# mlcolab/Pathfinder.jl

Hardware: AMD Instinct MI355X
Metric: ELBO draws/sec (multipathfinder hot path: fit + ELBO + pool + PSIS + resample) (higher is better)
Workload: dtype f64

## Files before the change

pathfinder.jl_amd/csrc/elbo_qf_kernel.hip:

```cpp
#include <type_traits>
#include <stdio.h>
#include <stdlib.h>
#include "pfmi_common.h"
#include "elbo_args.h"
#ifndef QF_PROF
#define QF_PROF 0
#endif

#ifndef QF_WAVES
#define QF_WAVES 8
#endif
#define QF_THREADS (QF_WAVES * 64)
#ifndef QF_NG
#define QF_NG 2
#endif
#ifndef QF_ABLATE
#define QF_ABLATE 0
#endif
#ifndef QF_NG2_MAXKC
#define QF_NG2_MAXKC 20
#endif
#ifndef QF_PRIO_FAIR
#define QF_PRIO_FAIR 8
#endif
#ifndef QF_PRIO_YOUNG
#define QF_PRIO_YOUNG 0
#endif
#ifndef QF_SETPRIO
#define QF_SETPRIO 0
#endif
#define QF_MIN_FRONT 1024
static_assert(QF_MIN_FRONT >= 2 * PF_ICDF_BFE_FRONT, "the look-up's front guard");
template <int KC> struct qf_chb { static constexpr int v = (KC > 20) ? 8 : 16; };

#pragma clang fp contract(off)

typedef double qf_d4 __attribute__((ext_vector_type(4)));
__device__ __forceinline__ qf_d4 qf_mfma16(double a, double b, qf_d4 c) { return __builtin_amdgcn_mfma_f64_16x16x4f64(a, b, c, 0, 0, 0); }
__device__ __forceinline__ double qf_mfma4(double a, double b, double c) { return __builtin_amdgcn_mfma_f64_4x4x4f64(a, b, c, 0, 0, 0); }

__host__ __device__ constexpr int qf_nconst(int KC, int RPAD) { return 4 + KC + KC * KC + RPAD + RPAD * KC + KC; }

template <int TGT>
__device__ __forceinline__ void qf_row_ac(const ElboArgs &A, const double *mu, int i, double &a, double &c) {
    if (TGT == 1) { a = A.t_a[i]; c = mu[i] - A.t_mean[i]; }
    else if (TGT == 2) { a = (i >= 1) ? 1.0 : 0.0; c = mu[i]; }
    else { a = 0.0; c = 0.0; }
}

template <int KC>
__device__ __forceinline__ int qf_vh_pos(int lrow, int col) {
    const int bl = lrow >> 4, rr = lrow & 15, q = rr >> 2, r = rr & 3, T = col >> 2, i = col & 3;
    return (((bl * 4 + r) * (KC / 4) + T) << 4) + q * 4 + i;
}

struct QfKernArgs { ElboArgs A; int ch_blocks, nchunks, groups_per_wg, ngroups, n_whole, n_tail, ndep; double *cshare; unsigned *cflag; unsigned epoch; };
#ifndef QF_SHARE_SPINS
#define QF_SHARE_SPINS 2000000
#endif
template <int KC, int TGT, int RPAD, int NG>
__global__ __launch_bounds__(QF_THREADS) void pf_elbo_qf_kernel(ElboArgs A, int ch_blocks, int nchunks, int groups_per_wg, int ngroups, int n_whole,
                                                                  int n_tail, int ndep, double *, unsigned *, unsigned) {
    extern __shared__ __attribute__((aligned(16))) double lds[];
#if QF_PROF
    const long long qf_t0 = wall_clock64();
    long long qf_tb = 0, qf_te = 0, qf_tp = 0, qf_last = 0;
#endif
    constexpr int NT = KC / 4, TR = RPAD / 4, NC = qf_nconst(KC, RPAD);
    constexpr int QF_CHB = qf_chb<KC>::v;
    constexpr bool FOLD = !(NG == 2 && KC >= 16);
    constexpr int PRE = (QF_CHB * 16 * KC + QF_THREADS - 1) / QF_THREADS;
    const int tid = threadIdx.x, wv = tid >> 6, lane = tid & 63, q = lane >> 4, c = lane & 15, l3 = lane & 3;
    const int d = A.d, nblk = (d + 15) >> 4;
    int slot = blockIdx.y, role = 0;
    int g_begin = blockIdx.x * groups_per_wg, g_cap = groups_per_wg;
    if (n_tail > 0 && slot >= n_whole) {
        constexpr int SL = QF_WAVES * NG, NPG_ = (TGT != 0) ? (KC + 1 + 15) / 16 : 0;
        int tail_f;
        if (slot < n_whole + n_tail) { role = 1; tail_f = slot - n_whole; g_begin = 0; g_cap = SL - NPG_; }
        else {
            const int t = slot - n_whole - n_tail;
            role = 2; tail_f = t / ndep;
            g_begin = (SL - NPG_) + (t - tail_f * ndep) * SL; g_cap = SL;
        }
        slot = n_whole + tail_f;
    }
    const int p = A.points[slot];
    const size_t blkidx = A.by_point ? (size_t)p : (size_t)slot;
    double *out_lp = A.logp + blkidx * A.log_stride, *out_lq = A.logq + blkidx * A.log_stride;
    constexpr int NPG = (TGT != 0) ? (KC + 1 + 15) / 16 : 0;
    const int npg = (role == 2) ? 0 : NPG;
    const int g_end = (g_begin + g_cap < ngroups) ? g_begin + g_cap : ngroups;
    const int nlb = (npg + (g_end - g_begin) + QF_WAVES * NG - 1) / (QF_WAVES * NG);
    if (A.status[p] != PFMI_FIT_OK) {
        for (int64_t n = (int64_t)g_begin * 16 + tid; n < (int64_t)g_end * 16 && n < A.N; n += QF_THREADS) {
            out_lp[n] = NAN; out_lq[n] = NAN;
        }
        return;
    }
    const int vh_sz = ch_blocks * 16 * KC, rs_sz = ch_blocks * 48;
    const int buf_stride = (nchunks > 1) ? vh_sz + rs_sz : 0;
    const int stage_sz = (nchunks > 1 ? 2 : 1) * (vh_sz + rs_sz);
    const int fix_off = stage_sz > QF_MIN_FRONT ? stage_sz : QF_MIN_FRONT;
    double *t_s = lds + fix_off;
    double *cn_s = t_s + KC * KC;
    double *g_s = cn_s + NC;
    double2 *icdf = reinterpret_cast<double2 *>(g_s + RPAD * RPAD + ((KC * KC + NC + RPAD * RPAD) & 1));

    const double *Vh = A.vh + (size_t)p * d * KC, *mu = A.mu + (size_t)p * d, *sqa = A.sqrt_alpha + (size_t)p * d;
    auto stage_direct = [&](int ck, int buf) {
        const int row0 = ck * ch_blocks * 16;
        double *vs = lds + buf * buf_stride, *rs = vs + vh_sz;
        const int npair = ch_blocks * 8 * KC;
        const int lim = (d - row0) * KC;
        const double2 *src = reinterpret_cast<const double2 *>(Vh + (size_t)row0 * KC);
        constexpr int U = 6;
        for (int j0 = tid; j0 < npair; j0 += QF_THREADS * U) {
            double2 v[U];
#pragma unroll
            for (int u = 0; u < U; ++u) {
                const int j = j0 + u * QF_THREADS, jc = (2 * j + 1 < lim) ? j : (lim >> 1) - 1;
                v[u] = src[jc];
            }
#pragma unroll
            for (int u = 0; u < U; ++u) {
                const int j = j0 + u * QF_THREADS, idx = 2 * j;
                if (j < npair) {
                    const int lrow = idx / KC, col = idx - lrow * KC;
                    const double2 val = (idx < lim) ? v[u] : make_double2(0.0, 0.0);
                    *reinterpret_cast<double2 *>(vs + qf_vh_pos<KC>(lrow, col)) = val;
                }
            }
        }
        for (int l0 = tid; l0 < ch_blocks * 16; l0 += QF_THREADS * 2) {
            double a[2], cc[2], s[2];
#pragma unroll
            for (int u = 0; u < 2; ++u) {
                const int lrow = l0 + u * QF_THREADS, row = row0 + lrow, rc = row < d ? row : d - 1;
                qf_row_ac<TGT>(A, mu, rc, a[u], cc[u]);
                s[u] = sqa[rc];
            }
#pragma unroll
            for (int u = 0; u < 2; ++u) {
                const int lrow = l0 + u * QF_THREADS, row = row0 + lrow;
                if (lrow < ch_blocks * 16) {
                    const bool in = row < d;
                    double *o = rs + (lrow >> 4) * 48 + (lrow & 15);
                    o[0] = in ? a[u] * s[u] * s[u] : 0.0; o[16] = in ? 2.0 * a[u] * cc[u] * s[u] : 0.0; o[32] = in ? s[u] : 0.0;
                }
            }
        }
    };
    {
        const double *T = A.tmat + (size_t)p * KC * KC;
        for (int i = tid; i < KC * KC; i += QF_THREADS) t_s[i] = T[i];
        for (int i = tid; i < NC; i += QF_THREADS) cn_s[i] = 0.0;
        if (RPAD > 0) for (int i = tid; i < RPAD * RPAD; i += QF_THREADS) g_s[i] = A.t_g[i];
        pf_icdf_load(icdf);
        stage_direct(0, 0);
    }
    const int rho = 4 * (c & 3) + (c >> 2);
    constexpr bool HREG = !(NG == 2 && KC >= 16);
    const double *Vc = A.vchol + (size_t)p * KC * KC;
    auto head_op = [&](const int which, const int r) -> double {
        const int b = 4 * q + r;
        if (which == 0) { double v = (rho == b) ? 1.0 : 0.0; if (rho < KC && b < KC) v = Vc[b * KC + rho]; return v; }
        const int i1 = 16 + rho, b1 = 16 + b;
        if (which == 1) return (i1 < KC) ? Vc[b * KC + i1] : 0.0;
        double v1 = (i1 == b1) ? 1.0 : 0.0;
        if (i1 < KC && b1 < KC) v1 = Vc[b1 * KC + i1];
        return v1;
    };
    double a_h00[HREG ? 4 : 1], a_h10[HREG ? 4 : 1], a_h11[HREG ? 4 : 1];
    if (HREG) {
#pragma unroll
        for (int r = 0; r < 4; ++r) {
            a_h00[HREG ? r : 0] = head_op(0, r);
            a_h10[HREG ? r : 0] = (KC > 16) ? head_op(1, r) : 0.0;
            a_h11[HREG ? r : 0] = (KC > 16) ? head_op(2, r) : 0.0;
        }
    }
    auto hop = [&](const int which, const int r) -> double {
        if (HREG) return which == 0 ? a_h00[HREG ? r : 0] : (which == 1 ? a_h10[HREG ? r : 0] : a_h11[HREG ? r : 0]);
        return head_op(which, r);
    };
    const uint64_t seed = A.seeds[slot];
    const uint32_t k0 = (uint32_t)seed, k1 = (uint32_t)(seed >> 32);
    const double logdet = A.logdet[p];
    __syncthreads();
#if QF_PROF
    qf_tp = wall_clock64() - qf_t0; qf_last = wall_clock64();
#endif
#if QF_PRIO_YOUNG
    if (wv >= 4) __builtin_amdgcn_s_setprio(1);
#endif
    if (TGT == 2) {
        if (tid == 0) { cn_s[1] = mu[0]; cn_s[2] = sqa[0]; }
        if (tid < KC) cn_s[4 + KC + KC * KC + RPAD + RPAD * KC + tid] = Vh[tid];
    }

    int cur = 0;
    for (int lb = 0; lb < nlb; ++lb) {
        bool pseudo[NG], active[NG];
        int sl[NG];
        int64_t nl[NG];
        uint32_t n[NG];
        double accw[NG][NT], acc3[NG][NT], acc4[NG][TR > 0 ? TR : 1];
        double usq[NG], q12[NG], z00[NG], u0[NG][4];
        bool any_active = false, any_pseudo = false, any_real = false;
#pragma unroll
        for (int g = 0; g < NG; ++g) {
            sl[g] = (lb * QF_WAVES + wv) * NG + g;
            pseudo[g] = sl[g] < npg;
            const int grp = g_begin + sl[g] - npg;
            active[g] = pseudo[g] || grp < g_end;
            nl[g] = (int64_t)grp * 16 + c;
            n[g] = (uint32_t)(A.n0 + nl[g]);
            any_active |= active[g]; any_pseudo |= pseudo[g]; any_real |= active[g] && !pseudo[g];
#pragma unroll
            for (int T = 0; T < NT; ++T) { accw[g][T] = 0.0; acc3[g][T] = 0.0; }
#pragma unroll
            for (int T = 0; T < (TR > 0 ? TR : 1); ++T) acc4[g][T] = 0.0;
            usq[g] = 0.0; q12[g] = 0.0; z00[g] = 0.0;
#pragma unroll
            for (int r = 0; r < 4; ++r) u0[g][r] = 0.0;
        }
        struct Pend { uint32_t x[4]; double dp[4]; double2 c01[4], c23[4]; };
        const uint32_t icdf_adj = pf_icdf_adj_bfe<PF_ICDF_NB_LDS>(icdf);
        auto gen_issue = [&](const int g, const int blk, Pend &P) {
#if QF_ABLATE == 1
#pragma unroll
            for (int r = 0; r < 4; ++r) { P.x[r] = 0x40000000u | (n[g] + blk); P.dp[r] = 1e-3 * (blk + r); P.c01[r] = make_double2(0.1, 0.2); P.c23[r] = make_double2(0.3, 0.4); }
#elif QF_ABLATE == 2
            pf_philox_normals(n[g], (uint32_t)(blk * 4 + q), 0u, 0u, k0, k1, P.x);
#pragma unroll
            for (int r = 0; r < 4; ++r) { P.dp[r] = (double)P.x[r] * 0x1p-32; P.c01[r] = make_double2(0.1, 0.2); P.c23[r] = make_double2(0.3, 0.4); }
#else
            pf_philox_normals(n[g], (uint32_t)(blk * 4 + q), 0u, 0u, k0, k1, P.x);
#pragma unroll
            for (int r = 0; r < 4; ++r) pf_icdf_issue_bfe<PF_ICDF_NB_LDS>(P.x[r], icdf_adj, P.dp[r], P.c01[r], P.c23[r]);
#endif
        };
        for (int ck = 0; ck < nchunks; ++ck) {
            double pre[PRE], pr_s = 0.0, pr_a = 0.0, pr_c = 0.0;
            const int nck = (ck + 1 < nchunks) ? ck + 1 : 0;
            const bool do_pre = (nchunks > 1) && (ck + 1 < nchunks || lb + 1 < nlb);
            if (do_pre) {
                const int row0 = nck * QF_CHB * 16;
                int tid_p = tid;
                asm volatile("" : "+v"(tid_p));
#pragma unroll
                for (int e = 0; e < PRE; ++e) {
                    const int idx = tid_p + e * QF_THREADS;
                    const int lrow = idx / KC, row = row0 + lrow;
                    pre[e] = (idx < QF_CHB * 16 * KC && row < d) ? Vh[(size_t)row0 * KC + idx] : 0.0;
                }
                if (tid_p < QF_CHB * 16) {
                    const int row = row0 + tid_p;
                    if (row < d) { qf_row_ac<TGT>(A, mu, row, pr_a, pr_c); pr_s = sqa[row]; }
                }
            }
            if (any_active) {
                const double *vs = lds + cur * buf_stride, *rs = vs + vh_sz;
                const int blk0 = ck * ch_blocks;
                const int nb = (nblk - blk0 < ch_blocks) ? nblk - blk0 : ch_blocks;
                struct Ops { double av[4][NT]; double wd[4][TR > 0 ? TR : 1]; double rs[12]; };
                auto load_ops = [&](const int bl, Ops &o) {
                    const double *rp = rs + bl * 48 + 4 * q;
                    const double *ap = vs + ((bl * 4) * NT << 4) + q * 4 + l3;
#pragma unroll
                    for (int r = 0; r < 4; ++r) {
#pragma unroll
                        for (int T = 0; T < NT; ++T) o.av[r][T] = ap[(r * NT + T) << 4];
                        o.rs[r] = rp[r]; o.rs[4 + r] = rp[16 + r]; o.rs[8 + r] = rp[32 + r];
                    }
                    if (TGT == 1 && RPAD > 0) {
                        const double *wp = A.t_wd16 + ((size_t)(blk0 + bl) * 16 + 4 * q) * 16 + l3;
#pragma unroll
                        for (int r = 0; r < 4; ++r)
#pragma unroll
                            for (int T = 0; T < TR; ++T) o.wd[r][T] = wp[r * 16 + 4 * T];
                    }
                };
                auto contract = [&](const int g, const double (&z)[4], const Ops &o, const bool with_w) {
#if QF_SETPRIO
                    __builtin_amdgcn_s_setprio(QF_SETPRIO);
#endif
                    double bp[4], bs[4];
#pragma unroll
                    for (int r = 0; r < 4; ++r) {
                        bp[r] = 0.0; bs[r] = 0.0;
                        if (TGT != 0) bp[r] = (with_w && FOLD) ? fma(o.rs[r], z[r], o.rs[4 + r]) : o.rs[r] * z[r];
                        if (TGT == 1 && RPAD > 0) bs[r] = o.rs[8 + r] * z[r];
                    }
                    __builtin_amdgcn_sched_barrier(0);
#pragma unroll
                    for (int r = 0; r < 4; ++r) {
                        if (TGT != 0) q12[g] = fma((with_w && FOLD) ? bp[r] : bp[r] + o.rs[4 + r], z[r], q12[g]);
#pragma unroll
                        for (int T = 0; T < NT; ++T) {
                            if (with_w) accw[g][T] = qf_mfma4(o.av[r][T], z[r], accw[g][T]);
                            if (TGT != 0) acc3[g][T] = qf_mfma4(o.av[r][T], bp[r], acc3[g][T]);
                        }
                        if (TGT == 1 && RPAD > 0) {
#pragma unroll
                            for (int T = 0; T < TR; ++T) acc4[g][T] = qf_mfma4(o.wd[r][T], bs[r], acc4[g][T]);
                        }
                    }
#if QF_SETPRIO
                    __builtin_amdgcn_s_setprio(0);
#endif
                };
                auto normals = [&](const int g, const int blk, double (&z)[4]) {
                    uint32_t x[4];
                    pf_philox_normals(n[g], (uint32_t)(blk * 4 + q), 0u, 0u, k0, k1, x);
                    pf_icdf4(x, n[g], (uint32_t)(blk * 4 + q), 0u, k0, k1, icdf, z);
                    if (blk == nblk - 1) {
#pragma unroll
                        for (int r = 0; r < 4; ++r) z[r] = (blk * 16 + 4 * q + r < d) ? z[r] : 0.0;
                    }
#pragma unroll
                    for (int r = 0; r < 4; ++r) usq[g] = fma(z[r], z[r], usq[g]);
                    if (blk == 0) {
                        qf_d4 h = {0.0, 0.0, 0.0, 0.0};
#pragma unroll
                        for (int r = 0; r < 4; ++r) { u0[g][r] = z[r]; h = qf_mfma16(hop(0, r), z[r], h); }
#pragma unroll
                        for (int r = 0; r < 4; ++r) z[r] = h[r];
                        z00[g] = z[0];
                    } else if (KC > 16 && blk == 1) {
                        qf_d4 h = {0.0, 0.0, 0.0, 0.0};
#pragma unroll
                        for (int r = 0; r < 4; ++r) h = qf_mfma16(hop(1, r), u0[g][r], h);
#pragma unroll
                        for (int r = 0; r < 4; ++r) h = qf_mfma16(hop(2, r), z[r], h);
#pragma unroll
                        for (int r = 0; r < 4; ++r) z[r] = h[r];
                    }
                };
                auto finish = [&](const int g, const int blk, const Pend &P, double (&z)[4], auto special_tag) {
                    constexpr bool SPECIAL = decltype(special_tag)::value;
#pragma unroll
                    for (int r = 0; r < 4; ++r) z[r] = pf_icdf_finish(P.x[r], P.dp[r], P.c01[r], P.c23[r]);
                    if (__builtin_expect(__any(pf_icdf_miss4(P.x)), 0))
                        pf_icdf4_fix(P.x, n[g], (uint32_t)(blk * 4 + q), 0u, k0, k1, z);
                    if (SPECIAL) {
                        if (blk == nblk - 1) {
#pragma unroll
                            for (int r = 0; r < 4; ++r) z[r] = (blk * 16 + 4 * q + r < d) ? z[r] : 0.0;
                        }
#pragma unroll
                        for (int r = 0; r < 4; ++r) usq[g] = fma(z[r], z[r], usq[g]);
                        if (blk == 0) {
                            qf_d4 h = {0.0, 0.0, 0.0, 0.0};
#pragma unroll
                            for (int r = 0; r < 4; ++r) { u0[g][r] = z[r]; h = qf_mfma16(hop(0, r), z[r], h); }
#pragma unroll
                            for (int r = 0; r < 4; ++r) z[r] = h[r];
                            z00[g] = z[0];
                        } else if (KC > 16 && blk == 1) {
                            qf_d4 h = {0.0, 0.0, 0.0, 0.0};
#pragma unroll
                            for (int r = 0; r < 4; ++r) h = qf_mfma16(hop(1, r), u0[g][r], h);
#pragma unroll
                            for (int r = 0; r < 4; ++r) h = qf_mfma16(hop(2, r), z[r], h);
#pragma unroll
                            for (int r = 0; r < 4; ++r) z[r] = h[r];
                        }
                    } else {
#pragma unroll
                        for (int r = 0; r < 4; ++r) usq[g] = fma(z[r], z[r], usq[g]);
                    }
                };
                auto pseudo_cols = [&](const int g, const int blk, const int bl, double (&z)[4]) {
                    const int j = 16 * sl[g] + c;
#pragma unroll
                    for (int r = 0; r < 4; ++r) {
                        const int row = blk * 16 + 4 * q + r;
                        double v = 0.0;
                        if (j < KC) v = vs[qf_vh_pos<KC>(bl * 16 + 4 * q + r, j)];
                        else if (j == KC && row < d) {
                            double aa, cc;
                            qf_row_ac<TGT>(A, mu, row, aa, cc);
                            v = cc / sqa[row];
                        }
                        z[r] = v;
                    }
                };
                if (any_pseudo) {
                    for (int bl = 0; bl < nb; ++bl) {
                        Ops oa;
                        load_ops(bl, oa);
#pragma unroll
                        for (int g = 0; g < NG; ++g) {
                            if (!active[g]) continue;
                            double z[4];
                            if (pseudo[g]) { pseudo_cols(g, blk0 + bl, bl, z); contract(g, z, oa, false); }
                            else { normals(g, blk0 + bl, z); contract(g, z, oa, true); }
                        }
                    }
                } else {
                    auto block_body_seq = [&](const int bl, auto special_tag) {
                        const int blk = blk0 + bl;
                        double z[NG][4];
#pragma unroll
                        for (int g = 0; g < NG; ++g) {
                            Pend pp;
                            gen_issue(g, blk, pp);
                            finish(g, blk, pp, z[g], special_tag);
                        }
                        const double *rp = rs + bl * 48 + 4 * q;
                        const double *ap = vs + ((bl * 4) * NT << 4) + q * 4 + l3;
#pragma unroll
                        for (int r = 0; r < 4; ++r) {
                            double av[NT];
#pragma unroll
                            for (int T = 0; T < NT; ++T) av[T] = ap[(r * NT + T) << 4];
                            const double r0 = rp[r], r1 = rp[16 + r];
#pragma unroll
                            for (int g = 0; g < NG; ++g) {
                                const double zr = z[g][r];
                                double bp = 0.0;
                                if (TGT != 0) {
                                    bp = r0 * zr;
                                    q12[g] = fma(bp + r1, zr, q12[g]);
                                }
#pragma unroll
                                for (int T = 0; T < NT; ++T) {
                                    accw[g][T] = qf_mfma4(av[T], zr, accw[g][T]);
                                    if (TGT != 0) acc3[g][T] = qf_mfma4(av[T], bp, acc3[g][T]);
                                }
                            }
                            if (TGT == 1 && RPAD > 0) {
                                const double *wp = A.t_wd16 + ((size_t)(blk0 + bl) * 16 + 4 * q + r) * 16 + l3;
                                double wd[TR > 0 ? TR : 1];
#pragma unroll
                                for (int T = 0; T < TR; ++T) wd[T] = wp[4 * T];
                                const double r2 = rp[32 + r];
#pragma unroll
                                for (int g = 0; g < NG; ++g) {
                                    const double bs = r2 * z[g][r];
#pragma unroll
                                    for (int T = 0; T < TR; ++T) acc4[g][T] = qf_mfma4(wd[T], bs, acc4[g][T]);
                                }
                            }
                        }
                    };
                    auto block_body = [&](const int bl, auto special_tag) {
                        if constexpr (NG == 2 && KC >= 16) { block_body_seq(bl, special_tag); return; }
                        const int blk = blk0 + bl;
                        Ops oa;
                        load_ops(bl, oa);
                        __builtin_amdgcn_sched_barrier(0);
                        Pend pp[NG];
                        double z[NG][4];
#pragma unroll
                        for (int g = 0; g < NG; ++g) gen_issue(g, blk, pp[g]);
#pragma unroll
                        for (int g = 0; g < NG; ++g) {
                            finish(g, blk, pp[g], z[g], special_tag);
#if QF_ABLATE == 3
                            q12[g] += z[g][0] + z[g][1] + z[g][2] + z[g][3] + oa.av[0][0] + oa.rs[0];
#else
                            contract(g, z[g], oa, true);
#endif
                        }
                    };
                    __builtin_amdgcn_s_waitcnt(0xC07F);
                    auto prio_turn = [&](const int blk) {
#if QF_PRIO_FAIR
                        if ((blk & (QF_PRIO_FAIR - 1)) == 0) {
                            if (((blk / QF_PRIO_FAIR) ^ (wv >> 2) ^ lb) & 1) __builtin_amdgcn_s_setprio(1); else __builtin_amdgcn_s_setprio(0);
                        }
#endif
                    };
                    if constexpr (NG == 2 && KC >= 16) {
                        for (int bl = 0; bl < nb; ++bl) {
                            const int blk = blk0 + bl;
                            prio_turn(blk);
                            if (__builtin_expect((blk == 0) | (blk == nblk - 1) | (KC > 16 && blk == 1), 0)) block_body(bl, std::true_type{});
                            else block_body(bl, std::false_type{});
                        }
                    } else {
                        constexpr int LEAD = (KC > 16) ? 2 : 1;
                        const int s_lo = (LEAD - blk0 <= 0) ? 0 : (LEAD - blk0 < nb ? LEAD - blk0 : nb);
                        const int s_hi = (blk0 + nb == nblk) ? (nb - 1 > s_lo ? nb - 1 : s_lo) : nb;
#pragma unroll
                        for (int bl = 0; bl < LEAD; ++bl)
                            if (bl < s_lo) { prio_turn(blk0 + bl); block_body(bl, std::true_type{}); }
                        for (int bl = s_lo; bl < s_hi; ++bl) { prio_turn(blk0 + bl); block_body(bl, std::false_type{}); }
                        if (s_hi < nb) { prio_turn(blk0 + s_hi); block_body(s_hi, std::true_type{}); }
                    }
                }
            }
            if (nchunks > 1) {
                if (do_pre) {
                    double *vs = lds + (cur ^ 1) * buf_stride, *rs = vs + vh_sz;
                    int tid_e = tid;
                    asm volatile("" : "+v"(tid_e));
#pragma unroll
                    for (int e = 0; e < PRE; ++e) {
                        const int idx = tid_e + e * QF_THREADS;
                        if (idx < QF_CHB * 16 * KC) { const int lrow = idx / KC; vs[qf_vh_pos<KC>(lrow, idx - lrow * KC)] = pre[e]; }
                    }
                    if (tid_e < QF_CHB * 16) {
                        double *o = rs + (tid_e >> 4) * 48 + (tid_e & 15);
                        o[0] = pr_a * pr_s * pr_s; o[16] = 2.0 * pr_a * pr_c * pr_s; o[32] = pr_s;
                    }
                }
                __syncthreads();
                cur ^= 1;
            }
        }
#if QF_PROF
        { const long long t_ = wall_clock64(); qf_tb += t_ - qf_last; qf_last = t_; }
#endif
        if (NPG > 0 && lb == 0) {
            int lane_p = lane;
            asm volatile("" : "+v"(lane_p));
            const int qp = lane_p >> 4, cp = lane_p & 15;
#pragma unroll
            for (int g = 0; g < NG; ++g) {
                if (!pseudo[g]) continue;
                const int j = 16 * sl[g] + cp;
                double *vv = cn_s + 4, *Mm = cn_s + 4 + KC, *t0 = Mm + KC * KC, *Nn = t0 + RPAD;
                const double q4 = pf_sum_q(q12[g]);
#pragma unroll
                for (int T = 0; T < NT; ++T) {
                    const int a = 4 * T + qp;
                    if (j < KC) Mm[a * KC + j] = acc3[g][T];
                    else if (j == KC) vv[a] = acc3[g][T];
                }
#pragma unroll
                for (int T = 0; T < TR; ++T) {
                    const int jr = 4 * T + qp;
                    if (j < KC) Nn[jr * KC + j] = acc4[g][T];
                    else if (j == KC) t0[jr] = acc4[g][T];
                }
                if (j == KC && qp == 0) cn_s[0] = q4 / 3.0;
            }
            double *cshare = nullptr; unsigned *cflag = nullptr; unsigned epoch = 0u; int tail_f = 0, n_tail_l = 0;
            if (role != 0) {
                const char *ka = (const char *)__builtin_amdgcn_kernarg_segment_ptr();
                asm volatile("" : "+s"(ka));
                cshare = *reinterpret_cast<double *const *>(ka + offsetof(QfKernArgs, cshare));
                cflag = *reinterpret_cast<unsigned *const *>(ka + offsetof(QfKernArgs, cflag));
                epoch = *reinterpret_cast<const unsigned *>(ka + offsetof(QfKernArgs, epoch));
                n_tail_l = *reinterpret_cast<const int *>(ka + offsetof(QfKernArgs, n_tail));
                const int n_whole_l = *reinterpret_cast<const int *>(ka + offsetof(QfKernArgs, n_whole));
                tail_f = slot - n_whole_l;
            }
            if (role == 2) {
                if (tid == 0) {
                    int spins = 0;
                    while (__hip_atomic_load(cflag + tail_f, __ATOMIC_ACQUIRE, __HIP_MEMORY_SCOPE_AGENT) != epoch && spins < QF_SHARE_SPINS) {
                        __builtin_amdgcn_s_sleep(32); ++spins;
                    }
                    if (spins >= QF_SHARE_SPINS) { cn_s[3] = NAN; atomicAdd(cflag + n_tail_l, 1u); }
                }
                __syncthreads();
                const bool lost = cn_s[3] != 0.0;
                const double *src = cshare + (size_t)tail_f * NC;
                double cv[(NC + QF_THREADS - 1) / QF_THREADS];
#pragma unroll
                for (int u = 0; u < (NC + QF_THREADS - 1) / QF_THREADS; ++u) {
                    const int i = tid + u * QF_THREADS;
                    cv[u] = __hip_atomic_load(src + (i < NC ? i : NC - 1), __ATOMIC_RELAXED, __HIP_MEMORY_SCOPE_AGENT);
                }
                __syncthreads();
#pragma unroll
                for (int u = 0; u < (NC + QF_THREADS - 1) / QF_THREADS; ++u) {
                    const int i = tid + u * QF_THREADS;
                    if (i < NC) cn_s[i] = lost ? NAN : cv[u];
                }
            }
            __syncthreads();
            if (role == 1) {
                double *dst = cshare + (size_t)tail_f * NC;
                for (int i = tid; i < NC; i += QF_THREADS) __hip_atomic_store(dst + i, cn_s[i], __ATOMIC_RELAXED, __HIP_MEMORY_SCOPE_AGENT);
                __threadfence();
                __syncthreads();
                if (tid == 0) __hip_atomic_store(cflag + tail_f, epoch, __ATOMIC_RELEASE, __HIP_MEMORY_SCOPE_AGENT);
            }
        }
        if (!any_real) continue;
        int lane_e = lane;
        asm volatile("" : "+v"(lane_e));
        const int qe = lane_e >> 4, ce = lane_e & 15;
#pragma unroll
        for (int g = 0; g < NG; ++g) {
            if (!active[g] || pseudo[g]) continue;
            double us = usq[g];
            us = pf_sum_q(us);
            double lp = NAN;
            if (TGT != 0) {
                double qs = q12[g];
                qs = pf_sum_q(qs);
                auto matvec = [&](const double *Mat, const int ld, const int nrows, auto nx_tag, auto ny_tag, auto lower_tag,
                                  const double (&x)[decltype(nx_tag)::value], double (&y)[decltype(ny_tag)::value]) {
                    constexpr int NX = decltype(nx_tag)::value, NY = decltype(ny_tag)::value;
                    constexpr bool LOWER = decltype(lower_tag)::value;
#pragma unroll
                    for (int rt = 0; rt < (NY + 3) / 4; ++rt) {
                        qf_d4 acc = {0.0, 0.0, 0.0, 0.0};
                        const int row = 16 * rt + ce;
#pragma unroll
                        for (int st = 0; st < NX; ++st) {
                            const int col = 4 * st + qe;
                            const bool ok = row < nrows && (!LOWER || col <= row);
                            const double av = ok ? Mat[row * ld + col] : 0.0;
                            acc = qf_mfma16(av, x[st], acc);
                        }
#pragma unroll
                        for (int r = 0; r < 4; ++r) if (4 * rt + r < NY) y[4 * rt + r] = acc[r];
                    }
                };
                const double *vv = cn_s + 4, *Mm = cn_s + 4 + KC, *t0 = Mm + KC * KC, *Nn = t0 + RPAD, *vh0 = Nn + RPAD * KC;
                double tvd[NT], mt[NT];
                matvec(t_s, KC, KC, std::integral_constant<int, NT>{}, std::integral_constant<int, NT>{}, std::false_type{}, accw[g], tvd);
                matvec(Mm, KC, KC, std::integral_constant<int, NT>{}, std::integral_constant<int, NT>{}, std::false_type{}, tvd, mt);
                double qa = 0.0;
#pragma unroll
                for (int T = 0; T < NT; ++T)
                    qa = fma(tvd[T], mt[T] - 2.0 * (FOLD ? acc3[g][T] - vv[4 * T + qe] : vv[4 * T + qe] + acc3[g][T]), qa);
                qa = pf_sum_q(qa);
                const double q1 = cn_s[0] + qs + qa;
                if (TGT == 1) {
                    double corr = 0.0;
                    if (RPAD > 0) {
                        constexpr int TRr = TR > 0 ? TR : 1;
                        double nt[TRr], tt[TRr], gg[TRr];
                        matvec(Nn, KC, RPAD, std::integral_constant<int, NT>{}, std::integral_constant<int, TRr>{}, std::false_type{}, tvd, nt);
#pragma unroll
                        for (int T = 0; T < TR; ++T) tt[T] = t0[4 * T + qe] + acc4[g][T] - nt[T];
                        matvec(g_s, RPAD, RPAD, std::integral_constant<int, TRr>{}, std::integral_constant<int, TRr>{}, std::true_type{}, tt, gg);
#pragma unroll
                        for (int T = 0; T < TR; ++T) corr = fma(gg[T], gg[T], corr);
                        corr = pf_sum_q(corr);
                    }
                    lp = A.t_offset - 0.5 * (q1 - corr);
                } else {
                    const double zh = __shfl(z00[g], ce, 64);
                    double pr = 0.0;
#pragma unroll
                    for (int T = 0; T < NT; ++T) pr = fma(vh0[4 * T + qe], tvd[T], pr);
                    pr = pf_sum_q(pr);
                    const double ta = cn_s[1] + cn_s[2] * (zh - pr), t3 = ta / 3.0;
                    lp = (t3 * t3 + (double)(d - 1) * ta + q1 * exp(-ta)) / -2.0;
                }
            }
            if (qe == 0 && nl[g] < A.N) {
                out_lq[nl[g]] = ((double)d * PF_LOG2PI + logdet + us) / -2.0;
                out_lp[nl[g]] = lp;
            }
        }
#if QF_PROF
        { const long long t_ = wall_clock64(); qf_te += t_ - qf_last; qf_last = t_; }
#endif
    }
#if QF_PROF
    if (g_begin == 0 && (slot & 1023) == 3 && lane == 0)
        printf("QF_PROF fit %d wave %d (10 ns ticks): prologue %lld blocks %lld epilogue+publish %lld total %lld batches %d\n", slot, wv, qf_tp, qf_tb,
               qf_te, (long long)(wall_clock64() - qf_t0), nlb);
#endif
}

static size_t qf_lds_bytes(int ch_blocks, int nchunks, int kc, int rpad) {
    const size_t per = (size_t)ch_blocks * 16 * kc + (size_t)ch_blocks * 48;
    size_t stage = per * (nchunks > 1 ? 2 : 1);
    if (stage < QF_MIN_FRONT) stage = QF_MIN_FRONT;
    return sizeof(double) * (stage + (size_t)kc * kc + qf_nconst(kc, rpad) + (size_t)rpad * rpad + 1 + 4 * PF_ICDF_LDS_ENTRIES + 2 * PF_ICDF_BFE_BEHIND);
}

static void qf_note_plan(pfmi_ctx *c, int kc, int tgt, int rpad, int ng, bool streamed, const char *cut) {
    char nm[64];
    snprintf(nm, sizeof nm, "qf:%d,%d,%d,%d:%s:%s", kc, tgt, rpad, ng, streamed ? "stream" : "res", cut);
    ++c->qf_plans[nm];
}

template <int KC, int TGT, int RPAD, int NG>
static int32_t launch_qf_ng(pfmi_ctx *c, const ElboArgs &a, int64_t nfits) {
    const int nblk = (a.d + 15) / 16;
    int ch_blocks = nblk, nchunks = 1;
    constexpr int QF_CHB = qf_chb<KC>::v;
    if (qf_lds_bytes(nblk, 1, KC, RPAD) > 156 * 1024) { ch_blocks = QF_CHB; nchunks = (nblk + QF_CHB - 1) / QF_CHB; }
    const size_t lds_bytes = qf_lds_bytes(ch_blocks, nchunks, KC, RPAD);
    PF_CHECK(lds_bytes <= 160 * 1024, PFMI_ERR_UNSUPPORTED, "qf kernel LDS %zu too large", lds_bytes);
    auto kern = pf_elbo_qf_kernel<KC, TGT, RPAD, NG>;
    PF_TRY(pf_raise_lds_limit(c, reinterpret_cast<const void *>(kern), 160 * 1024));
    const int ngroups = (int)((a.N + 15) / 16);
    constexpr int NPG = (TGT != 0) ? (KC + 1 + 15) / 16 : 0;
    int split = 1;
    while (!c->qf_seg_mode && (int64_t)split * nfits < 1024 && (ngroups + NPG) / (split * 2) >= QF_WAVES * NG) split *= 2;
    int gpw = (ngroups + split - 1) / split;
    if (split > 1) gpw = ((gpw + NPG + QF_WAVES * NG - 1) / (QF_WAVES * NG)) * (QF_WAVES * NG) - NPG;
    if (gpw < 1) gpw = 1;
    const int gx = (ngroups + gpw - 1) / gpw;
    auto launch = [&](int64_t f0, int64_t nf, int gpw_, int gx_) {
        for (int64_t s0 = f0; s0 < f0 + nf; s0 += 32768) {
            const int64_t ns = (f0 + nf - s0 < 32768) ? (f0 + nf - s0) : 32768;
            ElboArgs b = a;
            b.points = a.points + s0; b.seeds = a.seeds + s0;
            if (!a.by_point) { b.logp += s0 * a.log_stride; b.logq += s0 * a.log_stride; }
            hipLaunchKernelGGL(kern, dim3((unsigned)gx_, (unsigned)ns), dim3(QF_THREADS), lds_bytes, c->stream, b, ch_blocks, nchunks, gpw_,
                               ngroups, 0, 0, 0, (double *)nullptr, (unsigned *)nullptr, 0u);
        }
    };
    int64_t tail = 0;
    int gpw_t = gpw, gx_t = gx, ndep = 0;
    const char *no_tail = pf_debug_get("PFMI_QF_NO_TAIL");
    const char *two = pf_debug_get("PFMI_QF_TWO_LAUNCHES");
    const bool two_launches = (two && two[0] == '1') || c->qf_no_share;
    if (split == 1 && TGT != 0 && !(no_tail && no_tail[0] == '1') && !c->qf_seg_mode) {
        int ncu = 0;
        PF_HIP(hipDeviceGetAttribute(&ncu, hipDeviceAttributeMultiprocessorCount, c->device));
        if (c->ncu_eff > 0 && c->ncu_eff < ncu) ncu = c->ncu_eff;
        const int slots = QF_WAVES * NG, nb_full = (ngroups + NPG + slots - 1) / slots;
        const int64_t rem = ncu > 0 ? nfits % ncu : 0;
        gpw_t = slots - NPG;
        gx_t = gpw_t > 0 ? (ngroups + gpw_t - 1) / gpw_t : 0;
        ndep = (ngroups > gpw_t) ? (ngroups - gpw_t + slots - 1) / slots : 0;
        const bool share_ok = !two_launches && gpw_t > 0 && (nfits - rem) + rem * (1 + ndep) <= 65535;
        const int pieces = share_ok ? 1 + ndep : gx_t;
        if (rem > 0 && nfits > ncu && gpw_t > 0 && nb_full > 1 && (rem * pieces + ncu - 1) / ncu < nb_full) tail = rem;
        if (tail > 0 && share_ok) {
            constexpr int NC = qf_nconst(KC, RPAD);
            const size_t cbytes = (size_t)tail * NC * sizeof(double), fbytes = ((size_t)tail + 1) * sizeof(unsigned);
            DevBuf &share = c->qf_share_s[c->qf_slot];
            uint32_t &epoch = c->qf_epoch_s[c->qf_slot];
            if (share.cap < cbytes + fbytes || epoch == 0xFFFFFFFFu) {
                PF_CHECK(!c->stream_pending, PFMI_ERR_STATE, "scan: the hand-over buffer of a streaming call must be allocated before its first launch");
                PF_TRY(share.ensure(cbytes + fbytes + (64 << 10)));
                PF_HIP(hipMemsetAsync(share.p, 0, share.cap, c->stream));
                epoch = 0;
            }
            unsigned *cflag = reinterpret_cast<unsigned *>(share.as<char>() + share.cap) - (tail + 1);
            hipLaunchKernelGGL(kern, dim3(1, (unsigned)((nfits - tail) + tail * (1 + ndep))), dim3(QF_THREADS), lds_bytes, c->stream, a, ch_blocks,
                               nchunks, gpw, ngroups, (int)(nfits - tail), (int)tail, ndep, share.as<double>(), cflag, ++epoch);
            qf_note_plan(c, KC, TGT, RPAD, NG, nchunks > 1, "tail-share");
// ... 34 lines not shown
```

pathfinder.jl_amd/csrc/pfmi_common.h:

```cpp
#pragma once
#include <hip/hip_runtime.h>
#include <stdint.h>
#include <chrono>
#include <functional>
#include <memory>
#include <string>
#include <map>
#include <set>
#include <type_traits>
#include <vector>

#include "../../include/pfmi.h"
#include "pfmi_icdftab.h"

#define PF_LOG2PI 1.8378770664093454835606594728112352797227949472755668

void pf_set_error(const char *fmt, ...);
#define PF_HIP(call)                                                                              \
    do {                                                                                          \
        hipError_t e__ = (call);                                                                  \
        if (e__ != hipSuccess) {                                                                  \
            pf_set_error("%s failed: %s (%s:%d)", #call, hipGetErrorString(e__), __FILE__, __LINE__); \
            return PFMI_ERR_HIP;                                                                  \
        }                                                                                         \
// ... 236 lines not shown
int32_t pf_launch_fit(pfmi_ctx *c, int seg_l0 = 0, int seg_len = 0);
int32_t pf_launch_elbo_draws(pfmi_ctx *c, const int32_t *d_points, const uint64_t *d_seeds, int64_t nfits,
                             int64_t n0, int64_t N, const double *d_u, int64_t u_stride,
                             double *d_x, int64_t x_stride, double *d_logp, double *d_logq,
                             int64_t log_stride, bool with_target, bool by_point);
int32_t pf_launch_elbo_reduce(pfmi_ctx *c);
int32_t pf_launch_logpdf(pfmi_ctx *c, int64_t point, int64_t N, const double *d_x, double *d_out);
int32_t pf_launch_mixture_logpdf(pfmi_ctx *c, int K, const int32_t *d_points, int64_t N, const double *d_x, double *d_lse,
                                 double *d_comp);
int32_t pf_launch_psis(pfmi_ctx *c, const double *d_lr, int64_t S);
int32_t pf_launch_pool_moments(pfmi_ctx *c, int64_t col_offset, int importance, const double *d_center);
int32_t pf_launch_pool_cdf(pfmi_ctx *c, int64_t col_offset, int importance, int nthr, const double *d_thr, const double *d_carry);
int32_t pf_launch_pool_cross(pfmi_ctx *c, int64_t col_offset, int importance, const double *d_center, const double *d_carry);
int32_t pf_launch_pool_apply(pfmi_ctx *c, int64_t col_offset, int importance, const double *d_center, int r, const double *d_v,
                             const double *d_carry);
const char *pf_debug_get(const char *name);
void pf_comm_ctx_dying(pfmi_ctx *c);
int32_t pf_launch_resample(pfmi_ctx *c, int64_t S, int64_t ndraws, int importance, int replace,
                           uint64_t seed, const double *d_uniforms);
int32_t pf_enqueue_resample(pfmi_ctx *c, int64_t S, int64_t ndraws, int importance, int replace,
                            uint64_t seed, const double *d_uniforms);
int32_t pf_resample_check(pfmi_ctx *c);
int32_t pf_launch_pool_pick(pfmi_ctx *c, int have_fail_seeds);
int32_t pf_launch_nan_failed(pfmi_ctx *c, int64_t npts, int64_t N, const int32_t *d_points, double *d_lp);
int32_t pf_launch_resample_direct(pfmi_ctx *c, int64_t S, int64_t ndraws, const double *d_uniforms);
int32_t pf_launch_gather(pfmi_ctx *c, int64_t ndraws, const int64_t *d_idx, int64_t col_offset, double *d_out, bool skip_unowned = false);
int32_t pf_launch_gather_pos(pfmi_ctx *c, int64_t n, const int64_t *d_idx, const int64_t *d_pos, int64_t col_offset, double *d_out);
int32_t pf_launch_scatter_cols(pfmi_ctx *c, int64_t n, const int64_t *d_pos, const double *d_in, double *d_out);
int32_t pf_launch_idx_digest(pfmi_ctx *c, int64_t ndraws, const int64_t *d_idx, double *d_out4, double local_err);
int32_t pf_launch_logratio(pfmi_ctx *c, int64_t n);
int32_t pf_launch_scatter_rows(pfmi_ctx *c, int64_t ns, int64_t N, const int32_t *d_points, const double *d_src, double *d_dst);
int32_t pf_launch_lbfgs(pfmi_ctx *c, int K, int J, int maxiters, double g_tol, const double *d_x0, int pub_mask = -1, int32_t *h_prog = nullptr);
int32_t pf_launch_trace_pack(pfmi_ctx *c, int64_t cap);
size_t pf_lbc_path_state_bytes(int J);
int32_t pf_lbc_alloc(pfmi_ctx *c, int K, int J, int d);
int32_t pf_launch_lbc_init(pfmi_ctx *c, hipStream_t s);
int32_t pf_launch_lbc_step(pfmi_ctx *c, int64_t round, hipStream_t s);
int32_t pf_launch_woodbury_prim(pfmi_ctx *c, int mode, int64_t p, int64_t N, const double *d_in, double *d_out);
int32_t pf_launch_colsumsq(pfmi_ctx *c, int64_t N, const double *d_x, double *d_out);
int32_t pf_launch_woodbury_diag(pfmi_ctx *c, int64_t p, double *d_out);

inline int32_t pf_raise_lds_limit(pfmi_ctx *c, const void *kern, int bytes) {
    if (c->lds_attr_done.count(kern)) return PFMI_OK;
    PF_HIP(hipFuncSetAttribute(kern, hipFuncAttributeMaxDynamicSharedMemorySize, bytes));
    c->lds_attr_done.insert(kern);
    return PFMI_OK;
}

void pf_kernel_begin(pfmi_ctx *c);
void pf_kernel_end(pfmi_ctx *c, const char *name);

#ifdef __HIPCC__

__device__ __forceinline__ uint32_t pf_xor3_key(uint32_t a, uint32_t b, uint32_t k) {
    if (__builtin_constant_p(k)) return a ^ b ^ k;
    uint32_t r;
    asm("v_bitop3_b32 %0, %1, %2, %3 bitop3:0x96" : "=v"(r) : "v"(a), "v"(b), "s"(k));
    return r;
}
#define PF_NORMAL_ROUNDS 7
template <int ROUNDS>
__device__ __forceinline__ void pf_philox4x32(uint32_t c0, uint32_t c1, uint32_t c2, uint32_t c3,
                                              uint32_t k0, uint32_t k1, uint32_t (&out)[4]) {
#pragma unroll
    for (int r = 0; r < ROUNDS; ++r) {
        uint64_t p0 = (uint64_t)0xD2511F53u * c0;
        uint64_t p1 = (uint64_t)0xCD9E8D57u * c2;
        uint32_t n0 = pf_xor3_key((uint32_t)(p1 >> 32), c1, k0);
        uint32_t n1 = (uint32_t)p1;
        uint32_t n2 = pf_xor3_key((uint32_t)(p0 >> 32), c3, k1);
        uint32_t n3 = (uint32_t)p0;
        c0 = n0; c1 = n1; c2 = n2; c3 = n3;
        k0 += 0x9E3779B9u; k1 += 0xBB67AE85u;
    }
    out[0] = c0; out[1] = c1; out[2] = c2; out[3] = c3;
}
__device__ __forceinline__ void pf_philox_round(uint32_t &c0, uint32_t &c1, uint32_t &c2, uint32_t &c3,
                                                uint32_t &k0, uint32_t &k1) {
    const uint64_t p0 = (uint64_t)0xD2511F53u * c0;
    const uint64_t p1 = (uint64_t)0xCD9E8D57u * c2;
    const uint32_t n0 = (uint32_t)(p1 >> 32) ^ c1 ^ k0;
    const uint32_t n1 = (uint32_t)p1;
    const uint32_t n2 = (uint32_t)(p0 >> 32) ^ c3 ^ k1;
    const uint32_t n3 = (uint32_t)p0;
    c0 = n0; c1 = n1; c2 = n2; c3 = n3;
    k0 += 0x9E3779B9u; k1 += 0xBB67AE85u;
}
__device__ __forceinline__ void pf_philox4x32_10(uint32_t c0, uint32_t c1, uint32_t c2, uint32_t c3, uint32_t k0, uint32_t k1,
                                                 uint32_t (&out)[4]) {
    pf_philox4x32<10>(c0, c1, c2, c3, k0, k1, out);
}
__device__ __forceinline__ void pf_philox_normals(uint32_t c0, uint32_t c1, uint32_t c2, uint32_t c3, uint32_t k0, uint32_t k1,
                                                  uint32_t (&out)[4]) {
    pf_philox4x32<PF_NORMAL_ROUNDS>(c0, c1, c2, c3, k0, k1, out);
}

static __device__ const double PF_ICDF_TAB_DEV[PF_ICDF_ENTRIES][4] = { PF_ICDF_TABLE_ROWS };

template <int NB = PF_ICDF_NB_LDS>
__device__ __forceinline__ void pf_icdf_load(double2 *tab) {
    constexpr int NENT = NB << PF_ICDF_B;
    const double2 *src = reinterpret_cast<const double2 *>(&PF_ICDF_TAB_DEV[0][0]);
    for (int i0 = threadIdx.x; i0 < 2 * NENT; i0 += 4 * blockDim.x) {
        double2 v[4];
#pragma unroll
        for (int u = 0; u < 4; ++u) { const int i = i0 + u * (int)blockDim.x; v[u] = src[i < 2 * NENT ? i : 2 * NENT - 1]; }
#pragma unroll
        for (int u = 0; u < 4; ++u) { const int i = i0 + u * (int)blockDim.x; if (i < 2 * NENT) tab[(i & 1) * NENT + (NENT - 1 - (i >> 1))] = v[u]; }
    }
}
__device__ __forceinline__ double pf_icdf_any(uint32_t x, uint32_t x2) {
    const uint32_t mag = x & 0x7FFFFFFFu;
    double v;
    if (mag >= (1u << PF_ICDF_TAILBITS)) v = (double)mag;
    else v = ((double)(((uint64_t)mag << 32) | x2) + 0.5) * 0x1p-32;
    const unsigned hi = (unsigned)__double2hiint(v);
    const int idx = PF_ICDF_IDX0 - (int)(hi >> (20 - PF_ICDF_B));
    const double *c = PF_ICDF_TAB_DEV[idx];
// ... 304 lines not shown
```

Baseline: 506.6 million.

## Hoist per-draw Philox rounds out of the block loop and stage head operand in LDS

After: 515.1 million, median of 6. 1.02x the previous value.

```diff
diff --git a/pathfinder.jl_amd/csrc/elbo_qf_kernel.hip b/pathfinder.jl_amd/csrc/elbo_qf_kernel.hip
--- a/pathfinder.jl_amd/csrc/elbo_qf_kernel.hip
+++ b/pathfinder.jl_amd/csrc/elbo_qf_kernel.hip
@@ -17,6 +17,9 @@
 #ifndef QF_ABLATE
 #define QF_ABLATE 0
 #endif
+#ifndef QF_PHILOX_HOIST
+#define QF_PHILOX_HOIST 1
+#endif
 #ifndef QF_NG2_MAXKC
 #define QF_NG2_MAXKC 20
 #endif
@@ -40,6 +43,8 @@
 __device__ __forceinline__ double qf_mfma4(double a, double b, double c) { return __builtin_amdgcn_mfma_f64_4x4x4f64(a, b, c, 0, 0, 0); }
 
 __host__ __device__ constexpr int qf_nconst(int KC, int RPAD) { return 4 + KC + KC * KC + RPAD + RPAD * KC + KC; }
+
+__host__ __device__ constexpr int qf_head_lds(int KC, int NG) { return (NG == 2 && KC < 16) ? 256 : 0; }
 
 template <int TGT>
 __device__ __forceinline__ void qf_row_ac(const ElboArgs &A, const double *mu, int i, double &a, double &c) {
@@ -69,6 +74,7 @@
     constexpr int NT = KC / 4, TR = RPAD / 4, NC = qf_nconst(KC, RPAD);
     constexpr int QF_CHB = qf_chb<KC>::v;
     constexpr bool FOLD = !(NG == 2 && KC >= 16);
+    constexpr bool PHX = QF_PHILOX_HOIST != 0;
     constexpr int PRE = (QF_CHB * 16 * KC + QF_THREADS - 1) / QF_THREADS;
     const int tid = threadIdx.x, wv = tid >> 6, lane = tid & 63, q = lane >> 4, c = lane & 15, l3 = lane & 3;
     const int d = A.d, nblk = (d + 15) >> 4;
@@ -105,7 +111,8 @@
     double *t_s = lds + fix_off;
     double *cn_s = t_s + KC * KC;
     double *g_s = cn_s + NC;
-    double2 *icdf = reinterpret_cast<double2 *>(g_s + RPAD * RPAD + ((KC * KC + NC + RPAD * RPAD) & 1));
+    double *h_s = g_s + RPAD * RPAD;
+    double2 *icdf = reinterpret_cast<double2 *>(h_s + qf_head_lds(KC, NG) + ((KC * KC + NC + RPAD * RPAD) & 1));
 
     const double *Vh = A.vh + (size_t)p * d * KC, *mu = A.mu + (size_t)p * d, *sqa = A.sqrt_alpha + (size_t)p * d;
     auto stage_direct = [&](int ck, int buf) {
@@ -160,7 +167,8 @@
         stage_direct(0, 0);
     }
     const int rho = 4 * (c & 3) + (c >> 2);
-    constexpr bool HREG = !(NG == 2 && KC >= 16);
+    constexpr bool HLDS = qf_head_lds(KC, NG) > 0;
+    constexpr bool HREG = !(NG == 2 && KC >= 16) && !HLDS;
     const double *Vc = A.vchol + (size_t)p * KC * KC;
     auto head_op = [&](const int which, const int r) -> double {
         const int b = 4 * q + r;
@@ -180,7 +188,12 @@
             a_h11[HREG ? r : 0] = (KC > 16) ? head_op(2, r) : 0.0;
         }
     }
+    if (HLDS && wv == 0) {
+#pragma unroll
+        for (int r = 0; r < 4; ++r) h_s[r * 64 + lane] = head_op(0, r);
+    }
     auto hop = [&](const int which, const int r) -> double {
+        if (HLDS) return h_s[r * 64 + lane];
         if (HREG) return which == 0 ? a_h00[HREG ? r : 0] : (which == 1 ? a_h10[HREG ? r : 0] : a_h11[HREG ? r : 0]);
         return head_op(which, r);
     };
@@ -203,8 +216,9 @@
     for (int lb = 0; lb < nlb; ++lb) {
         bool pseudo[NG], active[NG];
         int sl[NG];
-        int64_t nl[NG];
-        uint32_t n[NG];
+        int grp[NG];
+        pf_philox_inv pinv[NG];
+        auto draw_of = [&](const int g) -> uint32_t { return (uint32_t)(A.n0 + ((int64_t)grp[g] * 16 + c)); };
         double accw[NG][NT], acc3[NG][NT], acc4[NG][TR > 0 ? TR : 1];
         double usq[NG], q12[NG], z00[NG], u0[NG][4];
         bool any_active = false, any_pseudo = false, any_real = false;
@@ -212,10 +226,12 @@
         for (int g = 0; g < NG; ++g) {
             sl[g] = (lb * QF_WAVES + wv) * NG + g;
             pseudo[g] = sl[g] < npg;
-            const int grp = g_begin + sl[g] - npg;
-            active[g] = pseudo[g] || grp < g_end;
-            nl[g] = (int64_t)grp * 16 + c;
-            n[g] = (uint32_t)(A.n0 + nl[g]);
+            grp[g] = g_begin + sl[g] - npg;
+            active[g] = pseudo[g] || grp[g] < g_end;
+            if (PHX) {
+                pinv[g] = pf_philox_draw_invariants(draw_of(g), k0, k1);
+                if constexpr (NG == 2 && KC >= 16) asm volatile("" : "+v"(pinv[g].C), "+v"(pinv[g].D), "+v"(pinv[g].E), "+v"(pinv[g].F));
+            }
             any_active |= active[g]; any_pseudo |= pseudo[g]; any_real |= active[g] && !pseudo[g];
 #pragma unroll
             for (int T = 0; T < NT; ++T) { accw[g][T] = 0.0; acc3[g][T] = 0.0; }
@@ -227,16 +243,20 @@
         }
         struct Pend { uint32_t x[4]; double dp[4]; double2 c01[4], c23[4]; };
         const uint32_t icdf_adj = pf_icdf_adj_bfe<PF_ICDF_NB_LDS>(icdf);
-        auto gen_issue = [&](const int g, const int blk, Pend &P) {
+        auto gen_issue = [&](const int g, const int blk, const uint64_t t, Pend &P) {
+            auto words = [&](uint32_t (&x)[4]) {
+                if (PHX) pf_philox4x32_hoisted<PF_NORMAL_ROUNDS>(pinv[g], t, k0, k1, x);
+                else pf_philox_normals(draw_of(g), (uint32_t)(blk * 4 + q), 0u, 0u, k0, k1, x);
+            };
 #if QF_ABLATE == 1
 #pragma unroll
-            for (int r = 0; r < 4; ++r) { P.x[r] = 0x40000000u | (n[g] + blk); P.dp[r] = 1e-3 * (blk + r); P.c01[r] = make_double2(0.1, 0.2); P.c23[r] = make_double2(0.3, 0.4); }
+            for (int r = 0; r < 4; ++r) { P.x[r] = 0x40000000u | (draw_of(g) + blk); P.dp[r] = 1e-3 * (blk + r); P.c01[r] = make_double2(0.1, 0.2); P.c23[r] = make_double2(0.3, 0.4); }
 #elif QF_ABLATE == 2
-            pf_philox_normals(n[g], (uint32_t)(blk * 4 + q), 0u, 0u, k0, k1, P.x);
+            words(P.x);
 #pragma unroll
             for (int r = 0; r < 4; ++r) { P.dp[r] = (double)P.x[r] * 0x1p-32; P.c01[r] = make_double2(0.1, 0.2); P.c23[r] = make_double2(0.3, 0.4); }
 #else
-            pf_philox_normals(n[g], (uint32_t)(blk * 4 + q), 0u, 0u, k0, k1, P.x);
+            words(P.x);
 #pragma unroll
             for (int r = 0; r < 4; ++r) pf_icdf_issue_bfe<PF_ICDF_NB_LDS>(P.x[r], icdf_adj, P.dp[r], P.c01[r], P.c23[r]);
 #endif
@@ -313,8 +333,8 @@
                 };
                 auto normals = [&](const int g, const int blk, double (&z)[4]) {
                     uint32_t x[4];
-                    pf_philox_normals(n[g], (uint32_t)(blk * 4 + q), 0u, 0u, k0, k1, x);
-                    pf_icdf4(x, n[g], (uint32_t)(blk * 4 + q), 0u, k0, k1, icdf, z);
+                    pf_philox_normals(draw_of(g), (uint32_t)(blk * 4 + q), 0u, 0u, k0, k1, x);
+                    pf_icdf4(x, draw_of(g), (uint32_t)(blk * 4 + q), 0u, k0, k1, icdf, z);
                     if (blk == nblk - 1) {
 #pragma unroll
                         for (int r = 0; r < 4; ++r) z[r] = (blk * 16 + 4 * q + r < d) ? z[r] : 0.0;
@@ -343,7 +363,7 @@
 #pragma unroll
                     for (int r = 0; r < 4; ++r) z[r] = pf_icdf_finish(P.x[r], P.dp[r], P.c01[r], P.c23[r]);
                     if (__builtin_expect(__any(pf_icdf_miss4(P.x)), 0))
-                        pf_icdf4_fix(P.x, n[g], (uint32_t)(blk * 4 + q), 0u, k0, k1, z);
+                        pf_icdf4_fix(P.x, draw_of(g), (uint32_t)(blk * 4 + q), 0u, k0, k1, z);
                     if (SPECIAL) {
                         if (blk == nblk - 1) {
 #pragma unroll
@@ -403,10 +423,11 @@
                     auto block_body_seq = [&](const int bl, auto special_tag) {
                         const int blk = blk0 + bl;
                         double z[NG][4];
+                        const uint64_t t = pf_philox_block_product((uint32_t)(blk * 4 + q), k0);
 #pragma unroll
                         for (int g = 0; g < NG; ++g) {
                             Pend pp;
-                            gen_issue(g, blk, pp);
+                            gen_issue(g, blk, t, pp);
                             finish(g, blk, pp, z[g], special_tag);
                         }
                         const double *rp = rs + bl * 48 + 4 * q;
@@ -454,8 +475,9 @@
                         __builtin_amdgcn_sched_barrier(0);
                         Pend pp[NG];
                         double z[NG][4];
-#pragma unroll
-                        for (int g = 0; g < NG; ++g) gen_issue(g, blk, pp[g]);
+                        const uint64_t t = pf_philox_block_product((uint32_t)(blk * 4 + q), k0);
+#pragma unroll
+                        for (int g = 0; g < NG; ++g) gen_issue(g, blk, t, pp[g]);
 #pragma unroll
                         for (int g = 0; g < NG; ++g) {
                             finish(g, blk, pp[g], z[g], special_tag);
@@ -560,17 +582,19 @@
                 }
                 __syncthreads();
                 const bool lost = cn_s[3] != 0.0;
+                int tid_s = tid;
+                asm volatile("" : "+v"(tid_s));
                 const double *src = cshare + (size_t)tail_f * NC;
                 double cv[(NC + QF_THREADS - 1) / QF_THREADS];
 #pragma unroll
                 for (int u = 0; u < (NC + QF_THREADS - 1) / QF_THREADS; ++u) {
-                    const int i = tid + u * QF_THREADS;
+                    const int i = tid_s + u * QF_THREADS;
                     cv[u] = __hip_atomic_load(src + (i < NC ? i : NC - 1), __ATOMIC_RELAXED, __HIP_MEMORY_SCOPE_AGENT);
                 }
                 __syncthreads();
 #pragma unroll
                 for (int u = 0; u < (NC + QF_THREADS - 1) / QF_THREADS; ++u) {
-                    const int i = tid + u * QF_THREADS;
+                    const int i = tid_s + u * QF_THREADS;
                     if (i < NC) cn_s[i] = lost ? NAN : cv[u];
                 }
             }
@@ -587,6 +611,11 @@
         int lane_e = lane;
         asm volatile("" : "+v"(lane_e));
         const int qe = lane_e >> 4, ce = lane_e & 15;
+        int wv_e = tid;
+        asm volatile("" : "+v"(wv_e));
+        wv_e >>= 6;
+        int d_e = d;
+        asm volatile("" : "+s"(d_e));
 #pragma unroll
         for (int g = 0; g < NG; ++g) {
             if (!active[g] || pseudo[g]) continue;
@@ -646,12 +675,13 @@
                     for (int T = 0; T < NT; ++T) pr = fma(vh0[4 * T + qe], tvd[T], pr);
                     pr = pf_sum_q(pr);
                     const double ta = cn_s[1] + cn_s[2] * (zh - pr), t3 = ta / 3.0;
-                    lp = (t3 * t3 + (double)(d - 1) * ta + q1 * exp(-ta)) / -2.0;
-                }
-            }
-            if (qe == 0 && nl[g] < A.N) {
-                out_lq[nl[g]] = ((double)d * PF_LOG2PI + logdet + us) / -2.0;
-                out_lp[nl[g]] = lp;
+                    lp = (t3 * t3 + (double)(d_e - 1) * ta + q1 * exp(-ta)) / -2.0;
+                }
+            }
+            const int64_t nl = (int64_t)(g_begin + (lb * QF_WAVES + wv_e) * NG + g - npg) * 16 + ce;
+            if (qe == 0 && nl < A.N) {
+                out_lq[nl] = ((double)d_e * PF_LOG2PI + logdet + us) / -2.0;
+                out_lp[nl] = lp;
             }
         }
 #if QF_PROF
@@ -665,11 +695,11 @@
 #endif
 }
 
-static size_t qf_lds_bytes(int ch_blocks, int nchunks, int kc, int rpad) {
+static size_t qf_lds_bytes(int ch_blocks, int nchunks, int kc, int rpad, int ng) {
     const size_t per = (size_t)ch_blocks * 16 * kc + (size_t)ch_blocks * 48;
     size_t stage = per * (nchunks > 1 ? 2 : 1);
     if (stage < QF_MIN_FRONT) stage = QF_MIN_FRONT;
-    return sizeof(double) * (stage + (size_t)kc * kc + qf_nconst(kc, rpad) + (size_t)rpad * rpad + 1 + 4 * PF_ICDF_LDS_ENTRIES + 2 * PF_ICDF_BFE_BEHIND);
+    return sizeof(double) * (stage + (size_t)kc * kc + qf_nconst(kc, rpad) + (size_t)rpad * rpad + qf_head_lds(kc, ng) + 1 + 4 * PF_ICDF_LDS_ENTRIES + 2 * PF_ICDF_BFE_BEHIND);
 }
 
 static void qf_note_plan(pfmi_ctx *c, int kc, int tgt, int rpad, int ng, bool streamed, const char *cut) {
@@ -683,8 +713,8 @@
     const int nblk = (a.d + 15) / 16;
     int ch_blocks = nblk, nchunks = 1;
     constexpr int QF_CHB = qf_chb<KC>::v;
-    if (qf_lds_bytes(nblk, 1, KC, RPAD) > 156 * 1024) { ch_blocks = QF_CHB; nchunks = (nblk + QF_CHB - 1) / QF_CHB; }
-    const size_t lds_bytes = qf_lds_bytes(ch_blocks, nchunks, KC, RPAD);
+    if (qf_lds_bytes(nblk, 1, KC, RPAD, NG) > 156 * 1024) { ch_blocks = QF_CHB; nchunks = (nblk + QF_CHB - 1) / QF_CHB; }
+    const size_t lds_bytes = qf_lds_bytes(ch_blocks, nchunks, KC, RPAD, NG);
     PF_CHECK(lds_bytes <= 160 * 1024, PFMI_ERR_UNSUPPORTED, "qf kernel LDS %zu too large", lds_bytes);
     auto kern = pf_elbo_qf_kernel<KC, TGT, RPAD, NG>;
     PF_TRY(pf_raise_lds_limit(c, reinterpret_cast<const void *>(kern), 160 * 1024));
diff --git a/pathfinder.jl_amd/csrc/pfmi_common.h b/pathfinder.jl_amd/csrc/pfmi_common.h
--- a/pathfinder.jl_amd/csrc/pfmi_common.h
+++ b/pathfinder.jl_amd/csrc/pfmi_common.h
@@ -312,18 +312,56 @@
 
 #ifdef __HIPCC__
 
-__device__ __forceinline__ uint32_t pf_xor3_key(uint32_t a, uint32_t b, uint32_t k) {
+__host__ __device__ __forceinline__ uint32_t pf_xor3_key(uint32_t a, uint32_t b, uint32_t k) {
+#if defined(__HIP_DEVICE_COMPILE__)
     if (__builtin_constant_p(k)) return a ^ b ^ k;
     uint32_t r;
     asm("v_bitop3_b32 %0, %1, %2, %3 bitop3:0x96" : "=v"(r) : "v"(a), "v"(b), "s"(k));
     return r;
+#else
+    return a ^ b ^ k;
+#endif
 }
 #define PF_NORMAL_ROUNDS 7
 template <int ROUNDS>
-__device__ __forceinline__ void pf_philox4x32(uint32_t c0, uint32_t c1, uint32_t c2, uint32_t c3,
+__host__ __device__ __forceinline__ void pf_philox4x32(uint32_t c0, uint32_t c1, uint32_t c2, uint32_t c3,
                                               uint32_t k0, uint32_t k1, uint32_t (&out)[4]) {
 #pragma unroll
     for (int r = 0; r < ROUNDS; ++r) {
+        uint64_t p0 = (uint64_t)0xD2511F53u * c0;
+        uint64_t p1 = (uint64_t)0xCD9E8D57u * c2;
+        uint32_t n0 = pf_xor3_key((uint32_t)(p1 >> 32), c1, k0);
+        uint32_t n1 = (uint32_t)p1;
+        uint32_t n2 = pf_xor3_key((uint32_t)(p0 >> 32), c3, k1);
+        uint32_t n3 = (uint32_t)p0;
+        c0 = n0; c1 = n1; c2 = n2; c3 = n3;
+        k0 += 0x9E3779B9u; k1 += 0xBB67AE85u;
+    }
+    out[0] = c0; out[1] = c1; out[2] = c2; out[3] = c3;
+}
+struct pf_philox_inv { uint32_t C, D, E, F; };
+__host__ __device__ __forceinline__ pf_philox_inv pf_philox_draw_invariants(uint32_t n, uint32_t k0, uint32_t k1) {
+    const uint64_t p = (uint64_t)0xD2511F53u * n;
+    const uint64_t r = (uint64_t)0xCD9E8D57u * ((uint32_t)(p >> 32) ^ k1);
+    const uint32_t A = (uint32_t)(r >> 32) ^ (k0 + 0x9E3779B9u);
+    const uint64_t s = (uint64_t)0xD2511F53u * A;
+    pf_philox_inv v;
+    v.C = (uint32_t)p ^ (k1 + 0xBB67AE85u);
+    v.D = (uint32_t)r ^ (k0 + 2u * 0x9E3779B9u);
+    v.E = (uint32_t)(s >> 32) ^ (k1 + 2u * 0xBB67AE85u);
+    v.F = (uint32_t)s;
+    return v;
+}
+__host__ __device__ __forceinline__ uint64_t pf_philox_block_product(uint32_t g, uint32_t k0) { return (uint64_t)0xD2511F53u * (g ^ k0); }
+template <int ROUNDS>
+__host__ __device__ __forceinline__ void pf_philox4x32_hoisted(const pf_philox_inv &v, uint64_t t, uint32_t k0, uint32_t k1, uint32_t (&out)[4]) {
+    static_assert(ROUNDS >= 3, "the hoisted form starts from the words after round 3");
+    const uint32_t t_lo = (uint32_t)t;
+    const uint64_t u = (uint64_t)0xCD9E8D57u * ((uint32_t)(t >> 32) ^ v.C);
+    uint32_t c0 = (uint32_t)(u >> 32) ^ v.D, c1 = (uint32_t)u, c2 = t_lo ^ v.E, c3 = v.F;
+    k0 += 3u * 0x9E3779B9u; k1 += 3u * 0xBB67AE85u;
+#pragma unroll
+    for (int r = 3; r < ROUNDS; ++r) {
         uint64_t p0 = (uint64_t)0xD2511F53u * c0;
         uint64_t p1 = (uint64_t)0xCD9E8D57u * c2;
         uint32_t n0 = pf_xor3_key((uint32_t)(p1 >> 32), c1, k0);
```
